# angelocatalani/neural-network-compression

Measured on AMD Instinct MI355X. Metric: weights/sec through prune+k-means (K=256), higher is better.
Workload: dtype f32

## Files before the change

### neural_network_compression_amd/csrc/nnc_hip.hip

```cpp
#include "nnc_common.hpp"
#include "nnc_km_shared.hpp"


extern "C" size_t nnc_kmeans_workspace_bytes(int32_t k)
{
    (void)k;
    return sizeof(KmWs) + 256;
}

extern "C" int32_t nnc_fix_shift(float absmax, int64_t n_total)
{
    int L = 1;
    while (((int64_t)1 << L) < n_total && L < 62) L++;
    if (!(absmax > 0.0f) || !std::isfinite(absmax)) return 0;
    int P = 0;
    (void)std::frexp((double)absmax, &P);
    return std::min(28, 62 - L) - P;
}

__device__ __forceinline__ int fix_f32(float v, int Sft)
{
    return (int)rintf(ldexpf(v, Sft));
}

// ... 1088 lines not shown
    if (__any(x) && (threadIdx.x & 63) == 0) *word = 1;
    km_lds_barrier();
    return *word;
}
__device__ __forceinline__ int km_vote_count(int *word, const int x)
{
    const int c = (int)__popcll(__ballot(x != 0));
    if (c && (threadIdx.x & 63) == 0) atomicAdd(word, c);
    km_lds_barrier();
    return *word;
}

template <int NT, bool MASS>
__device__ int km_finalize_relocate(KmWs *__restrict__ ws, const float *__restrict__ xs, const long long n, const KmTab *__restrict__ tab, const int ku,
                                    const int k, const int cur, long long *sum_o, long long *cnt_o, const float mean, const int Sft)
{
    constexpr int KC = NNC_KMAX;
    __shared__ __align__(16) unsigned char buf[sizeof(KlHead) + (size_t)KC * (8 + 8 + 4 + 4 + 4 + 4 + 2 + 2) + 4096 * 2];
    KlHead *hd = reinterpret_cast<KlHead *>(buf);
    KlArr L = {};
    {
        unsigned char *q = buf + sizeof(KlHead);
        L.A = reinterpret_cast<long long *>(q); q += (size_t)KC * 8;
        L.B = reinterpret_cast<long long *>(q); q += (size_t)KC * 8;
        L.cs = reinterpret_cast<float *>(q); q += (size_t)KC * 4;
        L.csq = reinterpret_cast<float *>(q); q += (size_t)KC * 4;
        L.cold = reinterpret_cast<float *>(q); q += (size_t)KC * 4;
        L.call = reinterpret_cast<float *>(q); q += (size_t)KC * 4;
        L.so = reinterpret_cast<uint16_t *>(q); q += (size_t)KC * 2;
        L.phi = reinterpret_cast<uint16_t *>(q); q += (size_t)KC * 2;
        L.qj = reinterpret_cast<uint16_t *>(q);
    }
    const int tid = threadIdx.x;
    if (tid == 0) { hd->n_empty = 0; hd->ku = ku; hd->nch = 0; hd->slow = 0; hd->r_flat = 0; }
    __syncthreads();
    int e = 0;
    for (int j = tid; j < k; j += NT) { e += cnt_o[j] == 0; L.cold[j] = ws->c[cur][j]; }
    if (e) atomicAdd(&hd->n_empty, e);
    __syncthreads();
    const bool mass = MASS && hd->n_empty > KL_RM_MAX;
    if (!MASS && hd->n_empty > KL_RM_MAX) return 0;
    if (!mass && 2 * ku > KL_RPASS * (NT / 8)) return 0;
    for (int p = tid; p < ku; p += NT) {
        const float2 c = tab->cand[p];
        L.cs[p] = c.x; L.csq[p] = c.y; L.so[p] = tab->orig[p];
        L.A[p] = ws->hint_a[p]; L.B[p] = ws->hint_b[p];
        const int ph = ws->bnd_phi[p];
        L.phi[p] = (uint16_t)(ph < p + 1 ? p + 1 : (ph > ku - 1 ? ku - 1 : ph));
    }
    __syncthreads();
    int *qfirst = reinterpret_cast<int *>(L.call);
    for (int j = tid; j + 1 < ku; j += NT) {
        const long long bm = j > 0 ? L.B[j - 1] : 0, a = L.A[j], b = L.B[j];
        const long long s0 = a > bm ? a : bm;
        const long long len = b - s0;
        qfirst[j] = 0;
        if (len > 0) {
            const int cs_ = (int)L.phi[j] == j + 1 ? KL_CHUNK : KL_CHUNK_CROWD;
            const long long nc = (len + cs_ - 1) / cs_;
            if (nc > (mass ? 512 : 64)) hd->slow = 1;
            else {
                const int first = atomicAdd(&hd->nch, (int)nc);
                qfirst[j] = first;
                for (int i = 0; i < (int)nc; i++) if (first + i < KL_QMAX) L.qj[first + i] = (uint16_t)j;
            }
        }
    }
    __syncthreads();
    if (NNC_FIN_TRACE_PTR && tid == 0) {
        unsigned long long *rt = NNC_FIN_TRACE_PTR;
        const int it = min(ws->st.iter, 63);
        rt[300 + 4 * it] = (unsigned long long)hd->n_empty; rt[301 + 4 * it] = (unsigned long long)hd->nch; rt[302 + 4 * it] = (unsigned long long)hd->slow; rt[303 + 4 * it] = (unsigned long long)ku;
    }
    if (hd->slow || hd->nch > 1024) return 0;
    if constexpr (MASS) {
        if (mass) {
            __shared__ KlMass mass_s;
            return kl_relocate_mass<NT>(xs, n, ws, hd, L, &mass_s, sum_o, cnt_o, k, hd->nch, mean, Sft);
        }
    }
    return kl_relocate<NT>(xs, n, ws, hd, L, sum_o, cnt_o, k, hd->nch, mean, Sft);
}

template <int NT, bool ONEWAVE, bool MASS = false>
__device__ __forceinline__ bool km_finalize_body(KmWs *__restrict__ ws, int mode, int resume, int *gcell, int *hcell, int *ku_out, const bool lazy = false,
                                                 const float *__restrict__ reloc_xs = nullptr, const long long reloc_n = 0, const int k_hint = 0)
{
    static_assert(!ONEWAVE || NT == 64, "the barrier-free form is for a single wave");
#define FIN_SYNC() do { if (ONEWAVE) wave_lds_fence(); else km_lds_barrier(); } while (0)
#define FIN_OR(slot, x) (ONEWAVE ? (int)__any(x) : km_vote_or(&fin_votes[slot], (x)))
#define FIN_AND(slot, x) (ONEWAVE ? (int)__all(x) : !km_vote_or(&fin_votes[slot], !(x)))
#define FIN_COUNT(slot, x) (ONEWAVE ? (int)__popcll(__ballot(x)) : km_vote_count(&fin_votes[slot], (x)))
    __shared__ int fin_votes[8];
    __shared__ long long sum_o[NNC_KMAX];
    __shared__ long long cnt_o[NNC_KMAX];
    __shared__ __align__(16) float cnew[NNC_KMAX];
    __shared__ float cs[NNC_KMAX];
    __shared__ uint16_t so[NNC_KMAX];
    __shared__ float sq[NNC_KMAX];
    __shared__ unsigned long long sh_key;
    __shared__ int ovf_n;
    __shared__ PwHeap heap;
    __shared__ float cu[NNC_KMAX];
    __shared__ uint16_t sou[NNC_KMAX];
    __shared__ double wave_a[NT / 64], wave_b[NT / 64];

    const int tid = threadIdx.x;
    unsigned long long *ftr = NNC_FIN_TRACE_PTR;
#define FSTAMP(i) do { if (ftr && tid == 0) ftr[i] = __builtin_amdgcn_s_memrealtime(); } while (0)
    FSTAMP(0);
    if (tid == 0) ws->cells_pending = 0;
    if (!ONEWAVE && tid < 8) fin_votes[tid] = 0;
    const int kb = k_hint > 0 ? min(k_hint, (int)NNC_KMAX) : (int)NNC_KMAX;
    const bool takes_a_pass = mode != FIN_FROM_PARTIALS;
    const bool from_shards = mode == FIN_FROM_SHARDS || mode == FIN_PACK_ONLY;
    const int qn_raw = takes_a_pass ? ws->q_n : 0;
    const int st_done = ws->st.done, st_paused = ws->st.paused, st_iter = ws->st.iter, reloc_fail = ws->reloc_fail;
    const int spec_go = ws->spec_go;
    const int k = ws->p.k, Sft = ws->p.fix_shift, max_iter = ws->p.max_iter, glog2 = ws->glog2;
    const float tol_v = ws->p.tol, p_lo = ws->p.lo, p_hi = ws->p.hi, inv_f = ws->inv;
    const long long n_tot = ws->p.n_total;
    const int ku0 = ws->tab[0].ku, ku1 = ws->tab[1].ku;
    int cur = ws->cur;
    const bool track = (mode == FIN_FROM_SHARDS) || (mode == FIN_FROM_PARTIALS && !resume);
    constexpr int RR = 2;
    long long pc[RR];
    float c_both[RR][2];
    uint16_t pm_both[RR][2], pmn_both[RR][2];
#pragma unroll
    for (int r = 0; r < RR; r++) {
        pc[r] = 0; c_both[r][0] = c_both[r][1] = 0.0f; pm_both[r][0] = pm_both[r][1] = pmn_both[r][0] = pmn_both[r][1] = 0;
        const int j = tid + r * NT;
        if (j < kb) {
            if (track) pc[r] = ws->prev_counts[j];
            if (mode != FIN_INIT) {
                c_both[r][0] = ws->c[0][j]; c_both[r][1] = ws->c[1][j];
                pm_both[r][0] = ws->tab[0].perm[j]; pm_both[r][1] = ws->tab[1].perm[j];
                if (j + 1 < NNC_KMAX) { pmn_both[r][0] = ws->tab[0].perm[j + 1]; pmn_both[r][1] = ws->tab[1].perm[j + 1]; }
            }
        }
    }
    long long sh_s[KM_NSHARD];
    unsigned long long sh_c[KM_NSHARD];
    uint16_t og_both[2] = {0, 0};
    const bool sh_pre = from_shards && tid < kb;
#pragma unroll
    for (int sh = 0; sh < KM_NSHARD; sh++) { sh_s[sh] = 0; sh_c[sh] = 0; }
    if (sh_pre) {
        og_both[0] = ws->tab[0].orig[tid]; og_both[1] = ws->tab[1].orig[tid];
#pragma unroll
        for (int sh = 0; sh < KM_NSHARD; sh++) { sh_s[sh] = ws->shard_sum[sh][tid]; sh_c[sh] = ws->shard_cnt[sh][tid]; }
    }
    const int qn = min(qn_raw, (int)NNC_KMAX);
    for (int r = tid; r < qn; r += NT) { ws->q_w0[r] = 0ull; ws->q_w1[r] = 0ull; ws->q_next[r] = 0; }
    FSTAMP(44);
#define FIN_QUEUE_RESET() do { if (tid == 0 && takes_a_pass) { ws->q_n = 0; ws->q_searched = 0; ws->help_hint = qn > 0; } } while (0)
#define FIN_LEAVE() do { if (ONEWAVE) wave_lds_fence(); else __syncthreads(); FIN_QUEUE_RESET(); return false; } while (0)
    if (mode != FIN_INIT && mode != FIN_PACK_ONLY && st_done) FIN_LEAVE();
    if (mode == FIN_FROM_SHARDS && st_paused) FIN_LEAVE();
    if (mode == FIN_PACK_ONLY && (st_done | st_paused)) {
        const int k2 = 2 * k;
        for (int i = tid; i < k2; i += NT) ws->partials[i] = ws->partials_local[i];
        FIN_LEAVE();
    }
    if (mode == FIN_FROM_PARTIALS && st_paused && !resume) FIN_LEAVE();
    if (resume == 2 && !spec_go) FIN_LEAVE();
    if (resume && reloc_fail) {
        if (tid == 0) ws->st.paused = 2;
        FIN_LEAVE();
    }

    float cold_r[RR];
    int spa[RR], spb[RR];
#pragma unroll
    for (int r = 0; r < RR; r++) {
        const int j = tid + r * NT;
        const bool in = mode != FIN_INIT && j < k;
        cold_r[r] = in ? (cur ? c_both[r][1] : c_both[r][0]) : 0.0f;
        spa[r] = in ? (int)(cur ? pm_both[r][1] : pm_both[r][0]) : 0;
        spb[r] = (in && j + 1 < k) ? (int)(cur ? pmn_both[r][1] : pmn_both[r][0]) : 0;
        if (!(track && j < k)) pc[r] = 0;
    }
    if (from_shards) {
        const KmTab *tab = &ws->tab[cur];
        const int ku_cur = cur ? ku1 : ku0;
        for (int j = tid; j < k; j += NT) { sum_o[j] = 0; cnt_o[j] = 0; }
        FIN_SYNC();
        FIN_QUEUE_RESET();
        FSTAMP(45);
        for (int p = tid; p < ku_cur; p += NT) {
            long long s = 0;
            unsigned long long c = 0;
            int o;
            if (p == tid && sh_pre) {
                o = cur ? og_both[1] : og_both[0];
#pragma unroll
                for (int sh = 0; sh < KM_NSHARD; sh++) { s += sh_s[sh]; c += sh_c[sh]; }
            } else {
                o = tab->orig[p];
                for (int sh = 0; sh < KM_NSHARD; sh++) { s += ws->shard_sum[sh][p]; c += ws->shard_cnt[sh][p]; }
            }
            for (int sh = 0; sh < KM_NSHARD; sh++) { ws->shard_sum[sh][p] = 0; ws->shard_cnt[sh][p] = 0; }
            sum_o[o] = s; cnt_o[o] = (long long)c;
        }
        FIN_SYNC();
        FSTAMP(46);
        for (int j = tid; j < k; j += NT) {
            ws->partials[j] = sum_o[j]; ws->partials[k + j] = cnt_o[j];
            ws->partials_local[j] = sum_o[j]; ws->partials_local[k + j] = cnt_o[j];
        }
        if (mode == FIN_PACK_ONLY) return false;
    } else if (mode == FIN_FROM_PARTIALS) {
        for (int j = tid; j < k; j += NT) { sum_o[j] = ws->partials[j]; cnt_o[j] = ws->partials[k + j]; }
    }
    FIN_SYNC();
    FSTAMP(47);
    if (!from_shards) FIN_QUEUE_RESET();
    int same_counts_now = 0;
    bool settled_event = false;
    if (track) {
        int count_diff = 0;
#pragma unroll
        for (int r = 0; r < RR; r++) {
            const int j = tid + r * NT;
            if (j < k) {
                const long long c = cnt_o[j];
                count_diff |= (pc[r] != c);
                ws->prev_counts[j] = c;
            }
        }
        const int any_diff = FIN_OR(0, count_diff);
        same_counts_now = any_diff ? 0 : 1;
        if (tid == 0) ws->st.same_counts = any_diff ? 0 : 1;
    }
    FSTAMP(1);

    if (mode != FIN_INIT) {
        int my_empty = 0;
        for (int j = tid; j < k; j += NT) my_empty += (cnt_o[j] == 0);
        if (tid == 0) sh_key = 0ull;
        int n_empty = FIN_COUNT(1, my_empty);
        bool settled = false;
        settled_event = false;
        if constexpr (!ONEWAVE) {
            if (n_empty > 0 && (MASS || n_empty <= KL_RM_MAX) && !resume && reloc_xs && mode == FIN_FROM_SHARDS && lazy && !(st_iter >= 1 && same_counts_now)) {
                __syncthreads();
                if (ftr && tid == 0) { ftr[20] = ftr[0]; ftr[21] = __builtin_amdgcn_s_memrealtime(); }
                const KmTab *tabc = &ws->tab[cur];
                settled = km_finalize_relocate<NT, MASS>(ws, reloc_xs, reloc_n, tabc, cur ? ku1 : ku0, k, cur, sum_o, cnt_o, ws->p.x_mean, Sft) != 0;
                if (settled) { n_empty = 0; settled_event = true; }
                if (settled && ftr && tid == 0) ftr[22] = __builtin_amdgcn_s_memrealtime();
            }
        }
        if (n_empty > 0 && !resume) {
            int tot_empty = 0;
            if (tid == 0) {
                for (int j = 0; j < k; j++) tot_empty += (cnt_o[j] == 0);
                ws->st.paused = 1; ws->st.n_empty = tot_empty;
                if (lazy) ws->tab[cur].n_ovf = 0;
            }
            return false;
        }
        for (int j = tid; j < k; j += NT)
            if (cnt_o[j] > 0) cnew[j] = (float)ldexp((double)sum_o[j] / (double)cnt_o[j], -Sft);
        FIN_SYNC();
        if (n_empty > 0) {
            for (int j = tid; j < k; j += NT)
                atomicMax(&sh_key, ((unsigned long long)cnt_o[j] << 11) | (unsigned long long)(2047 - j));
            FIN_SYNC();
            const int amax = 2047 - (int)(sh_key & 2047ull);
            for (int j = tid; j < k; j += NT)
                if (cnt_o[j] <= 0) {
                    cnew[j] = (amax < j) ? cnew[amax] : (float)ldexp((double)sum_o[amax], -Sft);
                }
            FIN_SYNC();
        }
        FSTAMP(2);
#pragma unroll
        for (int r = 0; r < RR; r++) {
            const int j = tid + r * NT;
            if (j < k) {
                float d = cnew[j] - cold_r[r];
                float s2 = d * d;
                float sft = (float)sqrt((double)s2);
                sq[j] = sft * sft;
            }
        }
        FIN_SYNC();
        float tot = 0.0f;
        if (ONEWAVE) tot = block_pairwise_sum<true>([&](int i) { return sq[i]; }, k, &heap);
        else if (tid < 64) tot = wave_pairwise_sum([&](int i) { return sq[i]; }, k, &heap);
        if (tid == 0) {
            int iter = st_iter + 1;
            int done = 0;
            if (tot <= tol_v) done = 1;
            else if (iter >= max_iter) done = 2;
            ws->st.iter = iter; ws->st.shift_tot = tot; ws->st.done = done;
            ws->st.paused = 0; ws->st.n_empty = 0;
            ws->cur = cur ^ 1;
        }
        cur ^= 1;
        for (int j = tid; j < k; j += NT) ws->c[cur][j] = cnew[j];
        FIN_SYNC();
    } else {
        for (int j = tid; j < k; j += NT) cnew[j] = ws->c[cur][j];
        FIN_SYNC();
    }

    FSTAMP(3);
    KmTab *tab = &ws->tab[cur];
    int still_sorted = 0;
    if (mode != FIN_INIT) {
        int ok = 1;
#pragma unroll
        for (int r = 0; r < RR; r++) {
            const int p = tid + r * NT;
            if (p < k) {
                const int a = spa[r];
                so[p] = (uint16_t)a;
                cs[p] = cnew[a];
                if (p + 1 < k) {
                    const int b = spb[r];
                    const float va = cnew[a], vb = cnew[b];
                    ok &= (va < vb) || (va == vb && a < b);
                }
            }
        }
        FSTAMP(12);
        still_sorted = FIN_AND(2, ok);
        const bool moved_far = resume || settled_event;
        for (int pass = 0; pass < 3 && !still_sorted && !moved_far; pass++) {
            for (int parity = 0; parity < 2; parity++) {
                for (int p = 2 * tid + parity; p + 1 < k; p += 2 * NT) {
                    const float va = cs[p], vb = cs[p + 1];
                    const uint16_t a = so[p], b = so[p + 1];
                    if (!((va < vb) || (va == vb && a < b))) { cs[p] = vb; cs[p + 1] = va; so[p] = b; so[p + 1] = a; }
                }
                FIN_SYNC();
            }
            int ok2 = 1;
            for (int p = tid; p + 1 < k; p += NT) {
                const float va = cs[p], vb = cs[p + 1];
                ok2 &= (va < vb) || (va == vb && so[p] < so[p + 1]);
            }
            still_sorted = FIN_AND(3 + pass, ok2);
        }
    }
    FSTAMP(8);
    if (ftr && tid == 0) ftr[13] = (unsigned long long)still_sorted;
    if (!still_sorted) {
        int parts = 1;
        while (parts < 64 && k * parts * 2 <= NT) parts <<= 1;
        const int per_part = (((k + parts - 1) / parts) + 3) & ~3;
        const float4 *c4 = reinterpret_cast<const float4 *>(cnew);
        for (int t = tid; t < ((k * parts + NT - 1) / NT) * NT; t += NT) {
            const int j = t / parts, part = t % parts;
            int rank = 0;
            float v = 0.0f;
            if (j < k) {
                v = cnew[j];
                const int i0 = part * per_part, i1 = min(k, i0 + per_part);
#pragma unroll 4
                for (int i = i0; i < i1; i += 4) {
                    const float4 u = c4[i >> 2];
                    rank += (int)(u.x < v) | ((int)(u.x == v) & (int)(i < j));
                    rank += ((int)(u.y < v) | ((int)(u.y == v) & (int)(i + 1 < j))) & (int)(i + 1 < i1);
                    rank += ((int)(u.z < v) | ((int)(u.z == v) & (int)(i + 2 < j))) & (int)(i + 2 < i1);
                    rank += ((int)(u.w < v) | ((int)(u.w == v) & (int)(i + 3 < j))) & (int)(i + 3 < i1);
                }
            }
            for (int off = 1; off < parts; off <<= 1) rank += __shfl_xor(rank, off);
            if (j < k && part == 0) { cs[rank] = v; so[rank] = (uint16_t)j; }
        }
    }
    FIN_SYNC();
    FSTAMP(9);
    if (settled_event && ftr && tid == 0) { ftr[23] = ftr[3]; ftr[24] = ftr[9]; }
    int ku = 0;
    {
        int *wave_i = reinterpret_cast<int *>(wave_a);
        const int rounds_u = (k + NT - 1) / NT;
        int carry = 0;
        for (int rd = 0; rd < rounds_u; rd++) {
            const int p = rd * NT + tid;
            float v = 0.0f;
            int o = 0, first = 0;
            if (p < k) {
                v = cs[p]; o = so[p];
                tab->perm[p] = (uint16_t)o;
                first = (p == 0) || (cs[p - 1] != v);
            }
            const unsigned long long bal = __ballot(first);
            const int before = __popcll(bal & ((1ull << (tid & 63)) - 1ull));
            if ((tid & 63) == 0) wave_i[tid >> 6] = __popcll(bal);
            FIN_SYNC();
            int pre = carry, tot = carry;
            for (int w = 0; w < NT / 64; w++) { const int wv = wave_i[w]; if (w < (tid >> 6)) pre += wv; tot += wv; }
            if (first) { cu[pre + before] = v; sou[pre + before] = (uint16_t)o; }
            carry = tot;
            FIN_SYNC();
        }
        ku = min(carry, k);
    }
    FSTAMP(10);
    for (int p = tid; p < ku; p += NT) {
        const float v = cu[p];
        cs[p] = v;
        tab->cand[p] = make_float2(v, v * v);
        tab->orig[p] = sou[p];
        ws->bnd.cand[p] = make_float2(v, v * v);
        ws->bnd.orig[p] = sou[p];
    }
    if (tid == 0) { tab->ku = ku; ws->ku_cur = ku; ws->bnd.ku = ku; ovf_n = 0; }
    FIN_SYNC();
    FSTAMP(4);
    const double U = 5.9604644775390625e-08;
    const double xb = fmax(fabs((double)p_lo), fabs((double)p_hi));
    const int G = 1 << glog2;
    const double lo = (double)p_lo;
    const double inv = (double)inv_f;
    const double ra = inv > 0.0 ? (1.0 - 4.0 * U) / inv * (1.0 - 4.0 * U) : 0.0;
    const double rb = inv > 0.0 ? (1.0 + 4.0 * U) / inv * (1.0 + 4.0 * U) : 0.0;
    {
        const int rounds = (ku + NT - 1) / NT;
        int *wave_i = reinterpret_cast<int *>(wave_a);
        int carry_g = -2;
        int wide_zone = 0;
        double *zhi = reinterpret_cast<double *>(sum_o), *zlo = reinterpret_cast<double *>(cnt_o);
// ... 1947 lines not shown
```

### neural_network_compression_amd/csrc/nnc_lloyd.hpp

```cpp

struct KlDiag { unsigned long long ph[16], last, sp[8], slast; };
#ifdef NNC_DIAG
#define KLSTAMP(slot) do { if (threadIdx.x == 0) { const unsigned long long now_ = __builtin_amdgcn_s_memrealtime(); dg->ph[slot] += now_ - dg->last; dg->last = now_; } } while (0)
#define KLSUB(slot) do { if (threadIdx.x == 0) { const unsigned long long now_ = __builtin_amdgcn_s_memrealtime(); dg->sp[slot] += now_ - dg->slast; dg->slast = now_; } } while (0)
#else
#define KLSTAMP(slot) do { } while (0)
#define KLSUB(slot) do { } while (0)
#endif
#define KL_MAXR 24
#define KL_TAIL_MAX 2048

struct KlHeap { int start[64]; int len[64]; float val[64]; };
struct KlHead {
    int ku, slow, nch, n_empty, depth, pad0, pad1, pad2;
    float tot;
    int f_empty, f_diff, f_reorder;
    int wave_i[16];
    double wmax[16], wmin[16];
    KlHeap heap;
    int r_cnt, r_bad, r_flat, r_pad1;
    unsigned long long r_keys[8];
    unsigned long long r_wkey[2][16];
    int r_widx[2][16];
    int r_empty[8], r_old[8];
};
static_assert(sizeof(KlHead) % 16 == 0, "the arrays behind the header are 16-byte aligned");

struct KlArr {
    double *Lb, *Ub;
    long long *sum_s, *cnt_s, *A, *B, *PA, *PB, *prevc, *hint;
    float *hL, *hR, *cs, *csq, *cnew, *cold, *sq, *call, *Lf, *Uf;
    uint16_t *so, *perm, *phi, *qj;
};

static size_t kl_lds_bytes(int kc) { return sizeof(KlHead) + (size_t)kc * (2 * 8 + 9 * 8 + 12 * 4 + 3 * 2) + 4096 * 2; }

__device__ __forceinline__ void kl_carve(unsigned char *smem, int kc, KlHead **hd, KlArr *L)
{
    *hd = reinterpret_cast<KlHead *>(smem);
    unsigned char *p = smem + sizeof(KlHead);
    auto take = [&](size_t bytes) { unsigned char *q = p; p += bytes; return q; };
    L->Lb = reinterpret_cast<double *>(take((size_t)kc * 8)); L->Ub = reinterpret_cast<double *>(take((size_t)kc * 8));
    L->sum_s = reinterpret_cast<long long *>(take((size_t)kc * 8)); L->cnt_s = reinterpret_cast<long long *>(take((size_t)kc * 8));
    L->A = reinterpret_cast<long long *>(take((size_t)kc * 8)); L->B = reinterpret_cast<long long *>(take((size_t)kc * 8));
    L->PA = reinterpret_cast<long long *>(take((size_t)kc * 8)); L->PB = reinterpret_cast<long long *>(take((size_t)kc * 8));
    L->prevc = reinterpret_cast<long long *>(take((size_t)kc * 8)); L->hint = reinterpret_cast<long long *>(take((size_t)kc * 16));
    L->hL = reinterpret_cast<float *>(take((size_t)kc * 8)); L->hR = reinterpret_cast<float *>(take((size_t)kc * 8));
    L->cs = reinterpret_cast<float *>(take((size_t)kc * 4)); L->csq = reinterpret_cast<float *>(take((size_t)kc * 4));
    L->cnew = reinterpret_cast<float *>(take((size_t)kc * 4)); L->cold = reinterpret_cast<float *>(take((size_t)kc * 4));
    L->sq = reinterpret_cast<float *>(take((size_t)kc * 4)); L->call = reinterpret_cast<float *>(take((size_t)kc * 4));
    L->Lf = reinterpret_cast<float *>(take((size_t)kc * 4)); L->Uf = reinterpret_cast<float *>(take((size_t)kc * 4));
    L->so = reinterpret_cast<uint16_t *>(take((size_t)kc * 2)); L->perm = reinterpret_cast<uint16_t *>(take((size_t)kc * 2));
    L->phi = reinterpret_cast<uint16_t *>(take((size_t)kc * 2));
    L->qj = reinterpret_cast<uint16_t *>(take((size_t)4096 * 2));
}

#define KL_DPP_I(v, ctrl) __builtin_amdgcn_update_dpp(0, (v), (ctrl), 0xF, 0xF, true)
#define KL_QP_XOR1 0xB1
#define KL_QP_XOR2 0x4E
#define KL_HALF_MIRROR 0x141
__device__ __forceinline__ int grp8_sum_i(int v)
{
    v += KL_DPP_I(v, KL_QP_XOR1); v += KL_DPP_I(v, KL_QP_XOR2); v += KL_DPP_I(v, KL_HALF_MIRROR);
    return v;
}
__device__ __forceinline__ int grp8_min_i(int v)
{
    v = min(v, KL_DPP_I(v, KL_QP_XOR1)); v = min(v, KL_DPP_I(v, KL_QP_XOR2)); v = min(v, KL_DPP_I(v, KL_HALF_MIRROR));
    return v;
}
__device__ __forceinline__ long long grp8_sum_ll(long long v)
{
#define KL_STEP_LL(ctrl) do { const int lo_ = KL_DPP_I((int)(unsigned)(v & 0xFFFFFFFFll), ctrl), hi_ = KL_DPP_I((int)(v >> 32), ctrl); \
        v += (long long)(((unsigned long long)(unsigned)hi_ << 32) | (unsigned)lo_); } while (0)
    KL_STEP_LL(KL_QP_XOR1); KL_STEP_LL(KL_QP_XOR2); KL_STEP_LL(KL_HALF_MIRROR);
#undef KL_STEP_LL
    return v;
}

__device__ void kl_heap_build(KlHead *hd, int n)
{
    KlHeap *hp = &hd->heap;
    const int lane = threadIdx.x & 63;
    hp->start[lane] = 0; hp->len[lane] = 0; hp->val[lane] = 0.0f;
    wave_lds_fence();
    if (lane == 0) { hp->start[1] = 0; hp->len[1] = n; }
    wave_lds_fence();
    int depth = 0;
    while (depth < 5 && ((n + (1 << depth) - 1) >> depth) > LEAF) depth++;
    if (depth < 5) depth++;
    for (int lev = 0; lev < depth; lev++) {
        const int i = (1 << lev) + lane;
        if (lane < (1 << lev)) {
            const int l = hp->len[i];
            if (l > LEAF) {
                int n2 = l / 2; n2 -= n2 % 8;
                hp->start[2 * i] = hp->start[i]; hp->len[2 * i] = n2;
                hp->start[2 * i + 1] = hp->start[i] + n2; hp->len[2 * i + 1] = l - n2;
            }
        }
        wave_lds_fence();
    }
    if (lane == 0) hd->depth = depth;
}

__device__ __forceinline__ float kl_leaf_sum(const float *e, int st, int l, int j8)
// ... 426 lines not shown
            const float xc = xs[s] - mean;
            float bestd = INFINITY;
            int best = j, besto = 0x7fffffff;
            for (int cc = j; cc <= (int)L.phi[j]; cc++) {
                const float d = L.csq[cc] + (-2.0f * (xc * L.cs[cc]));
                const int oc = (int)L.so[cc];
                if (d < bestd || (d == bestd && oc < besto)) { bestd = d; best = cc; besto = oc; }
            }
            atomicAdd(reinterpret_cast<unsigned long long *>(&L.sum_s[best]), (unsigned long long)((long long)fix_f32(xc, Sft) * len));
            atomicAdd(reinterpret_cast<unsigned long long *>(&L.cnt_s[best]), (unsigned long long)len);
            qfirst[j] = -1;
            hd->r_flat = 1;
        } else if (len > 0) {
            const int cs_ = (int)L.phi[j] == j + 1 ? KL_CHUNK : KL_CHUNK_CROWD;
            const long long nc = (len + cs_ - 1) / cs_;
            if (nc > KL_QONE) hd->slow = 1;
            else {
                const int first = atomicAdd(&hd->nch, (int)nc);
                qfirst[j] = first;
                for (int i = 0; i < (int)nc; i++) if (first + i < KL_QMAX) L.qj[first + i] = (uint16_t)j;
            }
        }
    }
}

template <int NT>
__device__ __forceinline__ void kl_label(const float *__restrict__ xs, const float mean, const int Sft, KlHead *hd, const KlArr &L)
{
    const int tid = threadIdx.x, g = tid >> 3, gl = tid & 7;
    const int nch = hd->nch;
    const int *qfirst = reinterpret_cast<const int *>(L.call);
    for (int c = g; c < nch; c += NT / 8) {
        const int j = (int)L.qj[c];
        const long long bm = j > 0 ? L.B[j - 1] : 0, a = L.A[j], e = L.B[j];
        const long long s = a > bm ? a : bm;
        const int phi = L.phi[j];
        const bool two = phi == j + 1;
        const int cs_ = two ? KL_CHUNK : KL_CHUNK_CROWD;
        const long long start = s + (long long)cs_ * (c - qfirst[j]);
        const long long end = start + cs_ < e ? start + cs_ : e;
        const float c0 = L.cs[j], q0 = L.csq[j], c1 = L.cs[j + 1], q1 = L.csq[j + 1];
        const bool tie1 = L.so[j + 1] < L.so[j];
        long long s0 = 0, s1 = 0;
        int n0 = 0, n1 = 0;
        for (long long r0 = start + gl; r0 < end; r0 += 64) {
            float v[8];
#pragma unroll
            for (int u = 0; u < 8; u++) { const long long r = r0 + 8 * u; v[u] = r < end ? xs[r] : 0.0f; }
#pragma unroll
            for (int u = 0; u < 8; u++) {
                if (r0 + 8 * u < end) {
                    const float xc = v[u] - mean;
                    const int q = fix_f32(xc, Sft);
                    if (two) {
                        const float d0 = q0 + (-2.0f * (xc * c0));
                        const float d1 = q1 + (-2.0f * (xc * c1));
                        if (d1 < d0 || (d1 == d0 && tie1)) { s1 += q; n1++; } else { s0 += q; n0++; }
                    } else {
                        float bestd = q0 + (-2.0f * (xc * c0));
                        int best = j, besto = (int)L.so[j];
                        for (int cc = j + 1; cc <= phi; cc++) {
                            const float d = L.csq[cc] + (-2.0f * (xc * L.cs[cc]));
                            const int oc = (int)L.so[cc];
                            if (d < bestd || (d == bestd && oc < besto)) { bestd = d; best = cc; besto = oc; }
                        }
                        atomicAdd(reinterpret_cast<unsigned long long *>(&L.sum_s[best]), (unsigned long long)(long long)q);
                        atomicAdd(reinterpret_cast<unsigned long long *>(&L.cnt_s[best]), 1ull);
                    }
                }
            }
        }
        const long long S0 = grp8_sum_ll(s0), S1 = grp8_sum_ll(s1);
        const int N01 = grp8_sum_i(n0 | (n1 << 16));
        if (gl == 0) {
            const int N0 = N01 & 0xFFFF, N1 = N01 >> 16;
            if (N0) { atomicAdd(reinterpret_cast<unsigned long long *>(&L.sum_s[j]), (unsigned long long)S0); atomicAdd(reinterpret_cast<unsigned long long *>(&L.cnt_s[j]), (unsigned long long)N0); }
            if (N1) { atomicAdd(reinterpret_cast<unsigned long long *>(&L.sum_s[j + 1]), (unsigned long long)S1); atomicAdd(reinterpret_cast<unsigned long long *>(&L.cnt_s[j + 1]), (unsigned long long)N1); }
        }
    }
}

#define KL_RW 8
#define KL_RM_MAX 7
#define KL_RKPT 16
#define KL_RPASS 10
template <int NT>
__device__ __forceinline__ int kl_relocate(const float *__restrict__ xs, const long long n, KmWs *__restrict__ ws, KlHead *hd, const KlArr &L,
                                           long long *sumo, long long *cnto, const int k, const int nch, const float mean, const int Sft)
{
    const int tid = threadIdx.x, lane = tid & 63, wv = tid >> 6, g = tid >> 3, gl = tid & 7;
    const int ku = hd->ku, m = hd->n_empty;
    if (tid == 0 && m > ws->kl_stats[7]) ws->kl_stats[7] = m;
    if (m < 1 || m > KL_RM_MAX || 2 * ku > KL_RPASS * (NT / 8) || hd->r_flat) { if (tid == 0) ws->kl_stats[6] |= 1; return 0; }
    unsigned long long *keys = ws->kl_keys;
    const int base = 2 * KL_RW * ku;
    unsigned long long *rtr = NNC_FIN_TRACE_PTR;
#define KRSTAMP(i) do { if (rtr && tid == 0) rtr[30 + (i)] = __builtin_amdgcn_s_memrealtime(); } while (0)
    KRSTAMP(0);
    if (tid == 0) { hd->r_cnt = 0; hd->r_bad = 0; }
    __syncthreads();
    unsigned inner = 0u;
    {
        long long rr[KL_RPASS];
        float xq[KL_RPASS];
        bool deep[KL_RPASS];
#pragma unroll
        for (int u = 0; u < KL_RPASS; u++) {
            const int q = g + u * (NT / 8);
            rr[u] = -1; deep[u] = false;
            if (q < 2 * ku) {
                const int p = q >> 1, side = q & 1;
                const long long lo_r = p > 0 ? L.B[p - 1] : 0, hi_r = p == ku - 1 ? n : L.A[p];
                long long r = -1;
                if (side == 0) { r = lo_r + gl; if (r >= hi_r) r = -1; }
                else { r = hi_r - 1 - gl; if (r < lo_r + KL_RW) r = -1; }
                rr[u] = r;
                deep[u] = gl == KL_RW - 1 && hi_r - lo_r > 2 * KL_RW;
            }
        }
#pragma unroll
        for (int u = 0; u < KL_RPASS; u++) xq[u] = rr[u] >= 0 ? xs[rr[u]] : 0.0f;
#pragma unroll
        for (int u = 0; u < KL_RPASS; u++) {
            const int q = g + u * (NT / 8);
            if (q < 2 * ku) {
                unsigned long long key = 0ull;
                if (rr[u] >= 0) {
                    const float dd = (xq[u] - mean) - L.cs[q >> 1];
                    const float dv = dd * dd;
                    key = ((unsigned long long)__float_as_uint(dv) << 32) | (unsigned long long)f32_ordered_bits(xq[u]);
                    if (deep[u]) inner = max(inner, __float_as_uint(dv));
                }
                keys[q * KL_RW + gl] = key;
            }
        }
    }
    KRSTAMP(1);
    const int *qfirst = reinterpret_cast<const int *>(L.call);
    for (int c = g; c < nch; c += NT / 8) {
        const int j = (int)L.qj[c];
        const long long bm = j > 0 ? L.B[j - 1] : 0, a = L.A[j], e = L.B[j];
        const long long s = a > bm ? a : bm;
        const int phi = L.phi[j];
        const int cs_ = phi == j + 1 ? KL_CHUNK : KL_CHUNK_CROWD;
        const long long start = s + (long long)cs_ * (c - qfirst[j]);
        const long long end = start + cs_ < e ? start + cs_ : e;
        int cbase = 0;
        if (gl == 0) cbase = atomicAdd(&hd->r_cnt, (int)(end - start));
        cbase = __shfl(cbase, (int)(threadIdx.x & 63 & ~7));
        for (long long r0 = start + gl; r0 < end; r0 += 64) {
            float xq[8];
#pragma unroll
            for (int u = 0; u < 8; u++) { const long long r = r0 + 8 * u; xq[u] = r < end ? xs[r] : 0.0f; }
#pragma unroll
            for (int u = 0; u < 8; u++) {
                if (r0 + 8 * u < end) {
                    const float xv = xq[u];
                    const float xc = xv - mean;
                    float bestd = L.csq[j] + (-2.0f * (xc * L.cs[j]));
                    int best = j, besto = (int)L.so[j];
                    for (int cc = j + 1; cc <= phi; cc++) {
                        const float d = L.csq[cc] + (-2.0f * (xc * L.cs[cc]));
                        const int oc = (int)L.so[cc];
                        if (d < bestd || (d == bestd && oc < besto)) { bestd = d; best = cc; besto = oc; }
                    }
                    const float dd = xc - L.cs[best];
                    const float dv = dd * dd;
                    const int slot = base + cbase + (int)(r0 + 8 * u - start);
                    if (slot < KL_RKEYS) keys[slot] = ((unsigned long long)__float_as_uint(dv) << 32) | (unsigned long long)f32_ordered_bits(xv);
                }
            }
        }
    }
    KRSTAMP(2);
    __syncthreads();
    KRSTAMP(3);
    const int N = base + hd->r_cnt;
    if (N > KL_RKPT * NT || N > KL_RKEYS) { if (tid == 0) ws->kl_stats[6] |= 2; return 0; }
    unsigned long long kr[KL_RKPT];
#pragma unroll
    for (int i = 0; i < KL_RKPT; i++) { const int slot = tid + i * NT; kr[i] = slot < N ? keys[slot] : 0ull; }
    KRSTAMP(4);
    if (tid <= KL_RM_MAX) hd->r_keys[tid] = 0ull;
#pragma unroll 1
    for (int r = 0; r <= m; r++) {
        {
            unsigned long long bk = 0ull;
            int bi = -1;
#pragma unroll
            for (int i = 0; i < KL_RKPT; i++) if (kr[i] > bk) { bk = kr[i]; bi = tid + i * NT; }
#pragma unroll
            for (int off = 32; off >= 1; off >>= 1) {
                const unsigned long long ok = (unsigned long long)__shfl_xor((long long)bk, off);
                const int oi = __shfl_xor(bi, off);
                if (ok > bk || (ok == bk && (unsigned)oi < (unsigned)bi)) { bk = ok; bi = oi; }
            }
            if (lane == 0) { hd->r_wkey[r & 1][wv] = bk; hd->r_widx[r & 1][wv] = bi; }
            __syncthreads();
            bk = 0ull; bi = -1;
#pragma unroll
            for (int w = 0; w < NT / 64; w++) {
                const unsigned long long ok = hd->r_wkey[r & 1][w];
                const int oi = hd->r_widx[r & 1][w];
                if (ok > bk || (ok == bk && (unsigned)oi < (unsigned)bi)) { bk = ok; bi = oi; }
            }
            if (tid == 0) hd->r_keys[r] = bk;
            if (bi >= 0 && (bi % NT) == tid) {
                const int mine = bi / NT;
#pragma unroll
                for (int i = 0; i < KL_RKPT; i++) if (i == mine) kr[i] = 0ull;
            }
        }
    }
    __syncthreads();
    KRSTAMP(5);
    const unsigned long long kcut = hd->r_keys[m - 1], ktop = hd->r_keys[0];
    int bad = 0;
    if (kcut == 0ull || (ktop >> 32) == 0ull) bad = 1;
    if (inner >= (unsigned)(kcut >> 32)) bad = 1;
    if (__syncthreads_or(bad)) { if (tid == 0) ws->kl_stats[6] |= (kcut == 0ull ? 4 : 0) | ((ktop >> 32) == 0ull ? 8 : 0) | 16; return 0; }
    {
        const int rounds = (k + NT - 1) / NT;
        int carry = 0;
        for (int rd = 0; rd < rounds; rd++) {
            const int j = rd * NT + tid;
            const int e = (j < k && cnto[j] == 0) ? 1 : 0;
            const unsigned long long bal = __ballot(e);
            const int before = __popcll(bal & ((1ull << lane) - 1ull));
            if (lane == 0) hd->wave_i[wv] = __popcll(bal);
            __syncthreads();
            int pre = carry, tot = carry;
            for (int w = 0; w < NT / 64; w++) { const int c = hd->wave_i[w]; if (w < wv) pre += c; tot += c; }
            if (e && pre + before < 8) hd->r_empty[pre + before] = j;
            carry = tot;
            __syncthreads();
        }
    }
    KRSTAMP(6);
    for (int i = wv; i < m; i += NT / 64) {
        const float xv = f32_from_ordered_bits((unsigned)(hd->r_keys[i] & 0xFFFFFFFFull));
        const float xc = xv - mean;
        float best = INFINITY;
        int old = 0x7fffffff;
        for (int j = lane; j < k; j += 64) {
            const float cv = L.cold[j];
            const float dj = cv * cv + (-2.0f * (xc * cv));
            if (dj < best) { best = dj; old = j; }
        }
#pragma unroll
        for (int off = 32; off >= 1; off >>= 1) {
            const float ob = __shfl_xor(best, off);
            const int oo = __shfl_xor(old, off);
            if (ob < best || (ob == best && oo < old)) { best = ob; old = oo; }
        }
        if (old == 0x7fffffff) old = 0;
        if (lane == 0) hd->r_old[i] = old;
    }
    __syncthreads();
    if (tid == 0) {
        int nb = 0;
        for (int i = 0; i < m; i++) {
            int leave = 0;
            for (int q = 0; q < m; q++) leave += hd->r_old[q] == hd->r_old[i];
            if (cnto[hd->r_old[i]] - leave < 1) nb = 1;
        }
        hd->r_bad = nb;
        if (nb) ws->kl_stats[6] |= 32;
        if (!nb) {
            for (int i = 0; i < m; i++) {
                const float xv = f32_from_ordered_bits((unsigned)(hd->r_keys[i] & 0xFFFFFFFFull));
                const long long v = (long long)fix_f32(xv - mean, Sft);
                const int old = hd->r_old[i], nw = hd->r_empty[i];
                sumo[old] -= v; cnto[old] -= 1;
                sumo[nw] += v; cnto[nw] += 1;
            }
            for (int i = 0; i < m; i++) {
                const int old = hd->r_old[i], nw = hd->r_empty[i];
                ws->partials[old] = sumo[old]; ws->partials[k + old] = cnto[old];
                ws->partials[nw] = sumo[nw]; ws->partials[k + nw] = cnto[nw];
            }
            if (m > 1) ws->st.reloc_multi += 1;
            const unsigned long long kn = hd->r_keys[m];
            if (kn != 0ull && (kn >> 32) == (kcut >> 32) && kn != kcut) ws->st.reloc_ties += 1;
            ws->st.n_relocated += 1;
            ws->st.n_in_place += 1;
            ws->reloc_fail = 0;
            ws->kl_stats[5] += 1;
        }
    }
    __syncthreads();
    KRSTAMP(7);
#undef KRSTAMP
    return hd->r_bad ? 0 : 1;
}

// ... 763 lines not shown
```

Before: 10.56 billion.

## Keep per-thread top-m keys in registers and insert moved centroids by binary search

The empty-cluster relocation no longer writes every candidate key to a global workspace and runs m+1 block-wide argmax rounds with a barrier each. Each thread now keeps a register top-(m+1) list, and a two-stage wave-then-block merge uses one barrier and no global key buffer. In finalize, when centroids have moved far because they were relocated or were previously empty, those few (at most 8) are pulled out, the rest are checked and fixed with odd-even passes, and the moved ones are placed by binary search and merged back. This avoids a full re-sort or slow path after relocation, at the cost of more complex ordering and tie-break logic.

```diff
diff --git a/neural_network_compression_amd/csrc/nnc_hip.hip b/neural_network_compression_amd/csrc/nnc_hip.hip
--- a/neural_network_compression_amd/csrc/nnc_hip.hip
+++ b/neural_network_compression_amd/csrc/nnc_hip.hip
@@ -1194,6 +1194,7 @@
     return kl_relocate<NT>(xs, n, ws, hd, L, sum_o, cnt_o, k, hd->nch, mean, Sft);
 }
 
+#define KM_MV_MAX 8
 template <int NT, bool ONEWAVE, bool MASS = false>
 __device__ __forceinline__ bool km_finalize_body(KmWs *__restrict__ ws, int mode, int resume, int *gcell, int *hcell, int *ku_out, const bool lazy = false,
                                                  const float *__restrict__ reloc_xs = nullptr, const long long reloc_n = 0, const int k_hint = 0)
@@ -1216,6 +1217,7 @@
     __shared__ float cu[NNC_KMAX];
     __shared__ uint16_t sou[NNC_KMAX];
     __shared__ double wave_a[NT / 64], wave_b[NT / 64];
+    __shared__ int mv_n, mv_pos[KM_MV_MAX], mv_idx[KM_MV_MAX], mv_rank[KM_MV_MAX];
 
     const int tid = threadIdx.x;
     unsigned long long *ftr = NNC_FIN_TRACE_PTR;
@@ -1223,6 +1225,7 @@
     FSTAMP(0);
     if (tid == 0) ws->cells_pending = 0;
     if (!ONEWAVE && tid < 8) fin_votes[tid] = 0;
+    if (!ONEWAVE && tid == 0) mv_n = 0;
     const int kb = k_hint > 0 ? min(k_hint, (int)NNC_KMAX) : (int)NNC_KMAX;
     const bool takes_a_pass = mode != FIN_FROM_PARTIALS;
     const bool from_shards = mode == FIN_FROM_SHARDS || mode == FIN_PACK_ONLY;
@@ -1244,7 +1247,7 @@
         pc[r] = 0; c_both[r][0] = c_both[r][1] = 0.0f; pm_both[r][0] = pm_both[r][1] = pmn_both[r][0] = pmn_both[r][1] = 0;
         const int j = tid + r * NT;
         if (j < kb) {
-            if (track) pc[r] = ws->prev_counts[j];
+            if (track || resume) pc[r] = ws->prev_counts[j];
             if (mode != FIN_INIT) {
                 c_both[r][0] = ws->c[0][j]; c_both[r][1] = ws->c[1][j];
                 pm_both[r][0] = ws->tab[0].perm[j]; pm_both[r][1] = ws->tab[1].perm[j];
@@ -1284,10 +1287,12 @@
 
     float cold_r[RR];
     int spa[RR], spb[RR];
+    unsigned was_empty = 0u;
 #pragma unroll
     for (int r = 0; r < RR; r++) {
         const int j = tid + r * NT;
         const bool in = mode != FIN_INIT && j < k;
+        if (resume && in && pc[r] == 0) was_empty |= 1u << r;
         cold_r[r] = in ? (cur ? c_both[r][1] : c_both[r][0]) : 0.0f;
         spa[r] = in ? (int)(cur ? pm_both[r][1] : pm_both[r][0]) : 0;
         spb[r] = (in && j + 1 < k) ? (int)(cur ? pmn_both[r][1] : pmn_both[r][0]) : 0;
@@ -1356,6 +1361,8 @@
         settled_event = false;
         if constexpr (!ONEWAVE) {
             if (n_empty > 0 && (MASS || n_empty <= KL_RM_MAX) && !resume && reloc_xs && mode == FIN_FROM_SHARDS && lazy && !(st_iter >= 1 && same_counts_now)) {
+#pragma unroll
+                for (int r = 0; r < RR; r++) if (tid + r * NT < k && cnt_o[tid + r * NT] == 0) was_empty |= 1u << r;
                 __syncthreads();
                 if (ftr && tid == 0) { ftr[20] = ftr[0]; ftr[21] = __builtin_amdgcn_s_memrealtime(); }
                 const KmTab *tabc = &ws->tab[cur];
@@ -1413,6 +1420,10 @@
         }
         cur ^= 1;
         for (int j = tid; j < k; j += NT) ws->c[cur][j] = cnew[j];
+        if (!ONEWAVE && (resume || settled_event)) {
+#pragma unroll
+            for (int r = 0; r < RR; r++) if (tid + r * NT < k) sou[tid + r * NT] = (uint16_t)(was_empty >> r & 1u);
+        }
         FIN_SYNC();
     } else {
         for (int j = tid; j < k; j += NT) cnew[j] = ws->c[cur][j];
@@ -1423,27 +1434,60 @@
     KmTab *tab = &ws->tab[cur];
     int still_sorted = 0;
     if (mode != FIN_INIT) {
+        const bool moved_far = resume || settled_event;
+        int m_ins = 0;
+        if (!ONEWAVE && moved_far) {
+#pragma unroll
+            for (int r = 0; r < RR; r++) {
+                const int p = tid + r * NT;
+                if (p < k && sou[spa[r]]) {
+                    const int slot = atomicAdd(&mv_n, 1);
+                    if (slot < KM_MV_MAX) { mv_pos[slot] = p; mv_idx[slot] = spa[r]; }
+                }
+            }
+            FIN_SYNC();
+            const int m = mv_n;
+            if (m >= 1 && m <= KM_MV_MAX && m < k) m_ins = m;
+        }
+        const int kk = k - m_ins;
         int ok = 1;
-#pragma unroll
-        for (int r = 0; r < RR; r++) {
-            const int p = tid + r * NT;
-            if (p < k) {
-                const int a = spa[r];
-                so[p] = (uint16_t)a;
-                cs[p] = cnew[a];
-                if (p + 1 < k) {
-                    const int b = spb[r];
-                    const float va = cnew[a], vb = cnew[b];
-                    ok &= (va < vb) || (va == vb && a < b);
+        if (m_ins) {
+#pragma unroll
+            for (int r = 0; r < RR; r++) {
+                const int p = tid + r * NT;
+                if (p < k && !sou[spa[r]]) {
+                    int before = 0;
+                    for (int i = 0; i < m_ins; i++) before += mv_pos[i] < p;
+                    so[p - before] = (uint16_t)spa[r];
+                    cs[p - before] = cnew[spa[r]];
+                }
+            }
+            FIN_SYNC();
+            for (int p = tid; p + 1 < kk; p += NT) {
+                const float va = cs[p], vb = cs[p + 1];
+                ok &= (va < vb) || (va == vb && so[p] < so[p + 1]);
+            }
+        } else {
+#pragma unroll
+            for (int r = 0; r < RR; r++) {
+                const int p = tid + r * NT;
+                if (p < k) {
+                    const int a = spa[r];
+                    so[p] = (uint16_t)a;
+                    cs[p] = cnew[a];
+                    if (p + 1 < k) {
+                        const int b = spb[r];
+                        const float va = cnew[a], vb = cnew[b];
+                        ok &= (va < vb) || (va == vb && a < b);
+                    }
                 }
             }
         }
         FSTAMP(12);
         still_sorted = FIN_AND(2, ok);
-        const bool moved_far = resume || settled_event;
-        for (int pass = 0; pass < 3 && !still_sorted && !moved_far; pass++) {
+        for (int pass = 0; pass < 3 && !still_sorted && (!moved_far || m_ins); pass++) {
             for (int parity = 0; parity < 2; parity++) {
-                for (int p = 2 * tid + parity; p + 1 < k; p += 2 * NT) {
+                for (int p = 2 * tid + parity; p + 1 < kk; p += 2 * NT) {
                     const float va = cs[p], vb = cs[p + 1];
                     const uint16_t a = so[p], b = so[p + 1];
                     if (!((va < vb) || (va == vb && a < b))) { cs[p] = vb; cs[p + 1] = va; so[p] = b; so[p + 1] = a; }
@@ -1451,11 +1495,53 @@
                 FIN_SYNC();
             }
             int ok2 = 1;
-            for (int p = tid; p + 1 < k; p += NT) {
+            for (int p = tid; p + 1 < kk; p += NT) {
                 const float va = cs[p], vb = cs[p + 1];
                 ok2 &= (va < vb) || (va == vb && so[p] < so[p + 1]);
             }
             still_sorted = FIN_AND(3 + pass, ok2);
+        }
+        if (m_ins && still_sorted) {
+            float tv[RR];
+            int to[RR];
+#pragma unroll
+            for (int r = 0; r < RR; r++) {
+                const int p = tid + r * NT;
+                tv[r] = 0.0f; to[r] = 0;
+                if (p < kk) { tv[r] = cs[p]; to[r] = so[p]; }
+            }
+            if (tid < m_ins) {
+                const int a = mv_idx[tid];
+                const float v = cnew[a];
+                int lo = 0, hi = kk;
+                while (lo < hi) {
+                    const int mid = (lo + hi) >> 1;
+                    const float u = cs[mid];
+                    if ((u < v) || (u == v && (int)so[mid] < a)) lo = mid + 1; else hi = mid;
+                }
+                mv_rank[tid] = lo;
+            }
+            FIN_SYNC();
+#pragma unroll
+            for (int r = 0; r < RR; r++) {
+                const int p = tid + r * NT;
+                if (p < kk) {
+                    int before = 0;
+                    for (int i = 0; i < m_ins; i++) before += mv_rank[i] <= p;
+                    cs[p + before] = tv[r]; so[p + before] = (uint16_t)to[r];
+                }
+            }
+            if (tid < m_ins) {
+                const int a = mv_idx[tid];
+                const float v = cnew[a];
+                int at = mv_rank[tid];
+                for (int i = 0; i < m_ins; i++) {
+                    const int b = mv_idx[i];
+                    const float u = cnew[b];
+                    at += (u < v) || (u == v && b < a);
+                }
+                cs[at] = v; so[at] = (uint16_t)a;
+            }
         }
     }
     FSTAMP(8);
diff --git a/neural_network_compression_amd/csrc/nnc_lloyd.hpp b/neural_network_compression_amd/csrc/nnc_lloyd.hpp
--- a/neural_network_compression_amd/csrc/nnc_lloyd.hpp
+++ b/neural_network_compression_amd/csrc/nnc_lloyd.hpp
@@ -20,8 +20,7 @@
     KlHeap heap;
     int r_cnt, r_bad, r_flat, r_pad1;
     unsigned long long r_keys[8];
-    unsigned long long r_wkey[2][16];
-    int r_widx[2][16];
+    unsigned long long r_wlist[16][8];
     int r_empty[8], r_old[8];
 };
 static_assert(sizeof(KlHead) % 16 == 0, "the arrays behind the header are 16-byte aligned");
@@ -614,7 +613,6 @@
 
 #define KL_RW 8
 #define KL_RM_MAX 7
-#define KL_RKPT 16
 #define KL_RPASS 10
 template <int NT>
 __device__ __forceinline__ int kl_relocate(const float *__restrict__ xs, const long long n, KmWs *__restrict__ ws, KlHead *hd, const KlArr &L,
@@ -624,47 +622,49 @@
     const int ku = hd->ku, m = hd->n_empty;
     if (tid == 0 && m > ws->kl_stats[7]) ws->kl_stats[7] = m;
     if (m < 1 || m > KL_RM_MAX || 2 * ku > KL_RPASS * (NT / 8) || hd->r_flat) { if (tid == 0) ws->kl_stats[6] |= 1; return 0; }
-    unsigned long long *keys = ws->kl_keys;
-    const int base = 2 * KL_RW * ku;
     unsigned long long *rtr = NNC_FIN_TRACE_PTR;
 #define KRSTAMP(i) do { if (rtr && tid == 0) rtr[30 + (i)] = __builtin_amdgcn_s_memrealtime(); } while (0)
     KRSTAMP(0);
-    if (tid == 0) { hd->r_cnt = 0; hd->r_bad = 0; }
-    __syncthreads();
+    if (tid == 0) hd->r_bad = 0;
+    if (tid <= KL_RM_MAX) hd->r_keys[tid] = 0ull;
+    __syncthreads();
+    unsigned long long top[KL_RM_MAX + 1];
+#pragma unroll
+    for (int i = 0; i <= KL_RM_MAX; i++) top[i] = 0ull;
+    auto keep = [&](unsigned long long key) {
+#pragma unroll
+        for (int i = 0; i <= KL_RM_MAX; i++) {
+            if (i > m) break;
+            const bool up = key > top[i];
+            const unsigned long long hi = up ? key : top[i];
+            key = up ? top[i] : key;
+            top[i] = hi;
+        }
+    };
+    float xe[KL_RPASS];
+    unsigned have = 0u, deep = 0u;
+#pragma unroll
+    for (int u = 0; u < KL_RPASS; u++) {
+        const int q = g + u * (NT / 8);
+        long long r = -1;
+        if (q < 2 * ku) {
+            const int p = q >> 1, side = q & 1;
+            const long long lo_r = p > 0 ? L.B[p - 1] : 0, hi_r = p == ku - 1 ? n : L.A[p];
+            if (side == 0) { r = lo_r + gl; if (r >= hi_r) r = -1; }
+            else { r = hi_r - 1 - gl; if (r < lo_r + KL_RW) r = -1; }
+            if (gl == KL_RW - 1 && hi_r - lo_r > 2 * KL_RW) deep |= 1u << u;
+        }
+        if (r >= 0) have |= 1u << u;
+        xe[u] = r >= 0 ? xs[r] : 0.0f;
+    }
     unsigned inner = 0u;
-    {
-        long long rr[KL_RPASS];
-        float xq[KL_RPASS];
-        bool deep[KL_RPASS];
-#pragma unroll
-        for (int u = 0; u < KL_RPASS; u++) {
-            const int q = g + u * (NT / 8);
-            rr[u] = -1; deep[u] = false;
-            if (q < 2 * ku) {
-                const int p = q >> 1, side = q & 1;
-                const long long lo_r = p > 0 ? L.B[p - 1] : 0, hi_r = p == ku - 1 ? n : L.A[p];
-                long long r = -1;
-                if (side == 0) { r = lo_r + gl; if (r >= hi_r) r = -1; }
-                else { r = hi_r - 1 - gl; if (r < lo_r + KL_RW) r = -1; }
-                rr[u] = r;
-                deep[u] = gl == KL_RW - 1 && hi_r - lo_r > 2 * KL_RW;
-            }
-        }
-#pragma unroll
-        for (int u = 0; u < KL_RPASS; u++) xq[u] = rr[u] >= 0 ? xs[rr[u]] : 0.0f;
-#pragma unroll
-        for (int u = 0; u < KL_RPASS; u++) {
-            const int q = g + u * (NT / 8);
-            if (q < 2 * ku) {
-                unsigned long long key = 0ull;
-                if (rr[u] >= 0) {
-                    const float dd = (xq[u] - mean) - L.cs[q >> 1];
-                    const float dv = dd * dd;
-                    key = ((unsigned long long)__float_as_uint(dv) << 32) | (unsigned long long)f32_ordered_bits(xq[u]);
-                    if (deep[u]) inner = max(inner, __float_as_uint(dv));
-                }
-                keys[q * KL_RW + gl] = key;
-            }
+#pragma unroll
+    for (int u = 0; u < KL_RPASS; u++) {
+        if (have >> u & 1u) {
+            const float dd = (xe[u] - mean) - L.cs[(g + u * (NT / 8)) >> 1];
+            const float dv = dd * dd;
+            keep(((unsigned long long)__float_as_uint(dv) << 32) | (unsigned long long)f32_ordered_bits(xe[u]));
+            if (deep >> u & 1u) inner = max(inner, __float_as_uint(dv));
         }
     }
     KRSTAMP(1);
@@ -677,9 +677,6 @@
         const int cs_ = phi == j + 1 ? KL_CHUNK : KL_CHUNK_CROWD;
         const long long start = s + (long long)cs_ * (c - qfirst[j]);
         const long long end = start + cs_ < e ? start + cs_ : e;
-        int cbase = 0;
-        if (gl == 0) cbase = atomicAdd(&hd->r_cnt, (int)(end - start));
-        cbase = __shfl(cbase, (int)(threadIdx.x & 63 & ~7));
         for (long long r0 = start + gl; r0 < end; r0 += 64) {
             float xq[8];
 #pragma unroll
@@ -698,51 +695,39 @@
                     }
                     const float dd = xc - L.cs[best];
                     const float dv = dd * dd;
-                    const int slot = base + cbase + (int)(r0 + 8 * u - start);
-                    if (slot < KL_RKEYS) keys[slot] = ((unsigned long long)__float_as_uint(dv) << 32) | (unsigned long long)f32_ordered_bits(xv);
+                    keep(((unsigned long long)__float_as_uint(dv) << 32) | (unsigned long long)f32_ordered_bits(xv));
                 }
             }
         }
     }
     KRSTAMP(2);
-    __syncthreads();
-    KRSTAMP(3);
-    const int N = base + hd->r_cnt;
-    if (N > KL_RKPT * NT || N > KL_RKEYS) { if (tid == 0) ws->kl_stats[6] |= 2; return 0; }
-    unsigned long long kr[KL_RKPT];
-#pragma unroll
-    for (int i = 0; i < KL_RKPT; i++) { const int slot = tid + i * NT; kr[i] = slot < N ? keys[slot] : 0ull; }
-    KRSTAMP(4);
-    if (tid <= KL_RM_MAX) hd->r_keys[tid] = 0ull;
 #pragma unroll 1
-    for (int r = 0; r <= m; r++) {
-        {
-            unsigned long long bk = 0ull;
-            int bi = -1;
-#pragma unroll
-            for (int i = 0; i < KL_RKPT; i++) if (kr[i] > bk) { bk = kr[i]; bi = tid + i * NT; }
+    for (int stage = 0; stage < 2; stage++) {
+        if (stage == 1) {
+            __syncthreads();
+#pragma unroll
+            for (int i = 0; i <= KL_RM_MAX; i++) top[i] = (lane < NT / 64 && i <= m) ? hd->r_wlist[lane][i] : 0ull;
+        }
+#pragma unroll 1
+        for (int r = 0; r <= m; r++) {
+            unsigned long long bk = top[0];
 #pragma unroll
             for (int off = 32; off >= 1; off >>= 1) {
                 const unsigned long long ok = (unsigned long long)__shfl_xor((long long)bk, off);
-                const int oi = __shfl_xor(bi, off);
-                if (ok > bk || (ok == bk && (unsigned)oi < (unsigned)bi)) { bk = ok; bi = oi; }
-            }
-            if (lane == 0) { hd->r_wkey[r & 1][wv] = bk; hd->r_widx[r & 1][wv] = bi; }
-            __syncthreads();
-            bk = 0ull; bi = -1;
-#pragma unroll
-            for (int w = 0; w < NT / 64; w++) {
-                const unsigned long long ok = hd->r_wkey[r & 1][w];
-                const int oi = hd->r_widx[r & 1][w];
-                if (ok > bk || (ok == bk && (unsigned)oi < (unsigned)bi)) { bk = ok; bi = oi; }
-            }
-            if (tid == 0) hd->r_keys[r] = bk;
-            if (bi >= 0 && (bi % NT) == tid) {
-                const int mine = bi / NT;
-#pragma unroll
-                for (int i = 0; i < KL_RKPT; i++) if (i == mine) kr[i] = 0ull;
-            }
-        }
+                bk = ok > bk ? ok : bk;
+            }
+            const unsigned long long holders = __ballot(top[0] == bk);
+            if (bk != 0ull && lane == __ffsll((long long)holders) - 1) {
+#pragma unroll
+                for (int i = 0; i < KL_RM_MAX; i++) top[i] = top[i + 1];
+                top[KL_RM_MAX] = 0ull;
+            }
+            if (lane == 0) {
+                if (stage == 0) hd->r_wlist[wv][r] = bk;
+                else if (wv == 0) hd->r_keys[r] = bk;
+            }
+        }
+        KRSTAMP(3 + stage);
     }
     __syncthreads();
     KRSTAMP(5);
```

After: 10.82 billion (median of 6 runs). 1.02x the previous value.
